# takahiroharada/OCLRadixSort

Hardware: AMD Instinct MI355X
Metric: Gkeys/s on uniform-random u32 keys; achieved % of HBM-read roofline (higher is better)
Workload: dtype u32; 1 GPU; Key-only RadixSort32, 67108864 uniform-random u32 keys (splitmix64 hi32, seed 123+step), 1xMI355X, in place; keys_per_gpu=67108864, parallelism=1 GPU, sort_algo=auto, digit_bits=8

## Files before the change

oclradixsort_amd/csrc/adlhip.hip:

```cpp
#include "../../include/adlhip.h"

#include <hip/hip_runtime.h>

#include <algorithm>
#include <cmath>
#include <cstdarg>
#include <cstdio>
#include <cstdlib>
#include <cstring>
#include <map>
#include <mutex>
#include <utility>
#include <string>
#include <vector>

#include "radix_kernels.hpp"
#include "onesweep_kernels.hpp"
#include "hybrid_kernels.hpp"
#include "persist_kernels.hpp"
#include "finish16_kernels.hpp"
#include "soa_wide_kernels.hpp"

#ifndef ADLHIP_SINGLE_TU
#define X(...) extern template __global__ __VA_ARGS__;
// ... 59 lines not shown
    uint64_t used_bytes = 0;
    int sort_algo = -1;
    int digit_bits = 8;
    int profile = 0;
    int tile_variant = -1;
    int rank_mode = 1;
    int lds_ordered = 0;
    int resident_wgs_device = 0;
    int resident_wgs = 0;
    int mid_path = 1;
    int mid_skip = 0;
    int mid2_skip = 0;
    int mid_backoff = 32, mid2_backoff = 64;
    int bin_finish = 1;
    int persist = 1;
    int msd2_path = 1;
    int net_lookback = 1;
    int partition_lookback = 1;
    int dict_path = 1;
    adlhip::DictBlock* d_dict = nullptr;
    uint32_t* d_msd2 = nullptr;
    std::vector<PendingProf> pending;
    std::vector<hipEvent_t> event_pool;
    std::map<std::string, ProfEntry> prof;
    std::vector<std::string> prof_order;
    std::vector<Staging> staging;
    std::vector<PinnedBlock> pinned_pool;
    size_t pinned_pool_bytes = 0;
    uint32_t* d_fault = nullptr;
    uint32_t* h_fault = nullptr;
// ... 524 lines not shown
    const size_t lds = std::max(own, (size_t)adlhip::TileCfg<E, 8, NT, K>::LDS_BYTES);
    if (ensure_lds(kern, lds)) return ADLHIP_FAILURE;
    const size_t per_cu = std::max<size_t>(1, std::min<size_t>((size_t)160 * 1024 / lds, (size_t)32 / (NT / 64)));
    const uint32_t grid = slab.state ? (uint32_t)num_segments
                                     : (uint32_t)std::min<size_t>(num_segments, per_cu * (size_t)d->prop.multiProcessorCount);
    return launch(d, sizeof(E) == 4 ? "segment_sort_u32" : "segment_sort_e64", [&] {
        hipLaunchKernelGGL(kern, dim3(grid), dim3(NT), lds, d->stream, in, out, seg_start, (uint32_t)num_segments, (uint32_t)low_bits,
                           dyn, d->d_fault, coop, slab);
    });
}

template <typename E, int K, typename S = E, bool SOA = false, int RANK = 1>
int launch_wave_segment_sort(adlhip_device* d, const E* in, E* out, const uint32_t* seg_start, size_t num_segments, int low_bits,
                             const uint32_t* seg_cnt = nullptr, uint32_t in_stride = 0, const uint32_t* gate = nullptr,
                             const uint32_t* dyn_low_bits = nullptr, uint32_t* out_vals = nullptr, const uint32_t* list = nullptr,
                             const uint32_t* list_cnt = nullptr, uint32_t seg_shift = 8)
{
    constexpr size_t per_wave = sizeof(E) * 64 * K + 256 * 4;
    constexpr int WAVES = per_wave <= 6144 ? 8    : per_wave <= 12288 ? 4 : per_wave <= 24576 ? 2 : 1;
    constexpr int STEP = K <= 40 ? 2 : 4;
    constexpr int RMIN = K <= 24 ? 2 : K / 2;
    const size_t lds = (size_t)WAVES * per_wave;
    if (list) {
        if constexpr (!SOA) {
            auto kern = adlhip::wave_segment_sort_kernel<E, K, WAVES, STEP, RMIN, S, SOA, true>;
            if (ensure_lds(kern, lds)) return ADLHIP_FAILURE;
            const size_t slots = std::min<size_t>(num_segments, (size_t)4 * d->prop.multiProcessorCount);
            const uint32_t grid = (uint32_t)((slots + WAVES - 1) / WAVES);
            return launch(d, sizeof(E) == 4 ? "segment_sort_listed_u32" : "segment_sort_listed_e64", [&] {
                hipLaunchKernelGGL(kern, dim3(grid), dim3(64 * WAVES), lds, d->stream, in, out, seg_start, (uint32_t)num_segments,
                                   (uint32_t)low_bits, d->d_fault, seg_cnt, in_stride, gate, dyn_low_bits, out_vals, list, list_cnt, seg_shift);
            });
        } else {
            return fail("internal: no list form for SoA");
        }
    }
    auto kern = adlhip::wave_segment_sort_kernel<E, K, WAVES, STEP, RMIN, S, SOA, false, RANK>;
    if (ensure_lds(kern, lds)) return ADLHIP_FAILURE;
    const uint32_t grid = (uint32_t)((num_segments + WAVES - 1) / WAVES);
    return launch(d, sizeof(E) == 4 ? "segment_sort_wave_u32" : "segment_sort_wave_e64", [&] {
        hipLaunchKernelGGL(kern, dim3(grid), dim3(64 * WAVES), lds, d->stream, in, out, seg_start, (uint32_t)num_segments,
                           (uint32_t)low_bits, d->d_fault, seg_cnt, in_stride, gate, dyn_low_bits, out_vals, list, list_cnt, seg_shift);
    });
}

template <typename E, typename S, int NT, int K, int BITS>
int launch_bin_segment_sort(adlhip_device* d, const S* in, E* out, const uint32_t* seg_off, const uint32_t* seg_cnt, uint32_t in_stride,
// ... 391 lines not shown
    L.off_mode = 0;
    L.off_cnt = L.off_mode + 256;
    L.off_off = L.off_cnt + 65536 * 4;
    L.off_hard = align_up(L.off_off + 65537 * 4, 256);
    L.off_coop = L.off_hard + 65536 * 4;
    L.off_slab_a = align_up(L.off_coop + kNetTableBytes, 256);
    L.off_slab_b = align_up(L.off_slab_a + (size_t)256 * L.stride_a * elem_bytes, 256);
    const size_t slab_b_bytes = (size_t)L.slots * L.stride_b * (elem_bytes == 4 && L.seg_shift == 8 ? 2 : elem_bytes);
    L.slab_b_in_tmp = elem_bytes == 4 && L.seg_shift == 8 && n >= kSlabInTmpMin && slab_b_bytes <= n * elem_bytes;
    L.total = L.off_slab_b + (L.slab_b_in_tmp ? 0 : slab_b_bytes);
    return L;
}

template <typename E, typename S, bool SOA = false>
int launch_large_finish(adlhip_device* d, const E* slab_b, E* out, uint32_t* out_vals, uint32_t* seg_off, uint32_t* seg_cnt, uint32_t stride_b,
                        uint32_t tier_b, uint32_t* mode, uint32_t* hard, int low_bits_max, bool bin, uint32_t seg_shift = 8);
bool use_bin_finish(const adlhip_device* d, size_t elem_bytes, bool key64, size_t n, bool whole_keys);

template <typename E>
int msd2_sort(adlhip_device* d, E* data, E* tmp, void* work, size_t n, int headroom_pct = kFullHeadroomPct)
{
    constexpr int K = sizeof(E) == 4 ? 32 : 16;
    constexpr int KEY_BITS = 8 * (int)sizeof(E);
    constexpr bool k32 = sizeof(E) == 4;
    uint32_t* cur_a = d->d_msd2;
    uint32_t* cur_b = d->d_msd2 + 8192;
    uint32_t* flag = d->d_msd2 + 8192 + 65536;
    uint32_t* done = flag + 1;
    uint32_t* sample = flag + 8;
    const Msd2Layout L = msd2_layout(n, sizeof(E), headroom_pct);
    char* wb = reinterpret_cast<char*>(work);
// ... 57 lines not shown
    using CC = adlhip::TileCfg<E, 8, 512, K>;
    auto ko = adlhip::msd2_offsets_kernel<E, 512, K>;
    if (ensure_lds(ko, CC::LDS_BYTES)) return ADLHIP_FAILURE;
    rc = launch(d, "msd2_offsets", [&] {
        hipLaunchKernelGGL(ko, dim3(net_wgs(d)), dim3(512), CC::LDS_BYTES, d->stream, cur_a, cur_b, flag, done, bar,
                           seg_cnt, seg_off, mode, (uint32_t)n, sample, data, tmp, ctable, d->d_fault, KEY_BITS,
                           8u - L.seg_shift, d->dict_path ? d->d_dict : nullptr, net_stats(d),
                           net_onesweep_args(d, wb + L.off_slab_a, (size_t)256 * L.stride_a * sizeof(E), n, 4, CC::TILE));
    });
    if (rc) return rc;
    using S = typename std::conditional<sizeof(E) == 4, uint16_t, E>::type;
    uint32_t* hard = reinterpret_cast<uint32_t*>(wb + L.off_hard);
    const int low_max = KEY_BITS - 8 - (int)L.seg_shift;
    const bool bin = use_bin_finish(d, sizeof(E), sizeof(E) == 8, L.seg_shift < 8 ? (size_t(24) << 20) : n, true);
    if (sizeof(E) == 4 && !slab16)
        return launch_large_finish<E, E>(d, slab_b, data, nullptr, seg_off, seg_cnt, L.stride_b, L.tier_b, mode, hard, low_max, bin, L.seg_shift);
    return launch_large_finish<E, S>(d, slab_b, data, nullptr, seg_off, seg_cnt, L.stride_b, L.tier_b, mode, hard, low_max, bin, L.seg_shift);
}

constexpr size_t kMsd2sAutoMin = size_t(1) << 20;
constexpr size_t kMsd2sMax = (size_t(1) << 28) + (size_t(1) << 22);
constexpr uint32_t msd2s_tile(size_t elem_bytes) { return elem_bytes == 8 ? 8192u : 16384u; }

struct Msd2sLayout {
    size_t off_mode, off_place, off_cnt, off_off, off_hard, off_coop, off_tickets, off_status_a, off_status_b, off_slab_a, off_slab_b, total;
    uint32_t pieces, slice, rows_a, rows_b, stride_a, stride_b, tier_b, ticket_words, seg_shift, slots;
    size_t status_bytes_a, status_bytes_b;
    bool slab_b_in_tmp;
};

Msd2sLayout msd2s_layout(size_t n, size_t elem_bytes = 8, bool slab16 = false, bool lean = false)
{
// ... 56 lines not shown
    const bool forced = d->msd2_path >= 2;
    const bool whole = sort_bits == max_bits;
    if (d->rank_mode != 1 && (keys || n > (size_t(96) << 20) || msd2_tier_b(n, 256u << msd2_seg_shift(n, false)) > 2560u)) return kLargeNone;
    if (!keys) return n > (forced ? kMsd2Min : kMsd2sAutoMin) && n <= kMsd2sMax ? kLargeStable : kLargeNone;
    if (n <= (forced || elem_bytes == 8 ? kMsd2Min : kMsd2AutoMin)) return kLargeNone;
    const size_t cursor_max = elem_bytes == 4 ? kMsd2MaxU32 : kMsd2MaxU64;
    if (!whole || d->msd2_path == 3) return n <= kMsd2sMax ? kLargeStable : kLargeNone;
    if (d->msd2_path == 4) return n <= cursor_max ? kLargeCursor : kLargeNone;
    if (d->msd2_path == 5) return n <= kMsd2sMax ? kLargeHybrid : kLargeNone;
    const size_t hybrid_min = d->persist ? (size_t(192) << 20) : (size_t(96) << 20);
    if (elem_bytes == 4 && n >= hybrid_min && n <= kMsd2sMax) return kLargeHybrid;
    if (elem_bytes == 8 && n >= (size_t(48) << 20) && n <= kMsd2sMax) return kLargeStable;
    return n <= cursor_max ? kLargeCursor : kLargeNone;
}

template <typename E, typename S, bool SOA>
int launch_large_finish(adlhip_device* d, const E* slab_b, E* out, uint32_t* out_vals, uint32_t* seg_off, uint32_t* seg_cnt, uint32_t stride_b,
                        uint32_t tier_b, uint32_t* mode, uint32_t* hard, int low_bits_max, bool bin, uint32_t seg_shift)
{
    const uint32_t* lowb = mode + adlhip::kDynLowBits;
    const size_t slots = (size_t)256 << seg_shift;
    constexpr bool wg_kind = !SOA && sizeof(E) == 4 && sizeof(S) == 2;
    if constexpr (wg_kind) {
        if (d->persist && !bin && seg_shift == 8 && tier_b <= 2560 && (stride_b & 1u) == 0u) {
            const uint16_t* sb = reinterpret_cast<const uint16_t*>(slab_b);
#define ADLHIP_F16(R2_, WAVES_)                                                                                                      \
    {                                                                                                                                \
        auto kf = adlhip::wave_finish16_kernel<R2_, WAVES_, true, true, 1>;                                                                   \
        const size_t lds = (size_t)WAVES_ * adlhip::Finish16Cfg<R2_>::PER_WAVE;                                                      \
        if (ensure_lds(kf, lds)) return ADLHIP_FAILURE;                                                                              \
        return launch(d, "segment_sort_wave_u32", [&] {                                                                              \
            hipLaunchKernelGGL(kf, dim3((uint32_t)((slots + WAVES_ - 1) / WAVES_)), dim3(64 * WAVES_), lds, d->stream, sb, out, seg_off,       \
                               seg_cnt, stride_b, mode, lowb, (uint32_t)slots, d->d_fault);                                          \
        });                                                                                                                          \
    }
            if (tier_b <= 1280) ADLHIP_F16(10, 4)
            if (tier_b <= 1536) ADLHIP_F16(12, 4)
            ADLHIP_F16(20, 4)
#undef ADLHIP_F16
        }
    }
    static const uint32_t wg_min = getenv("ADLHIP_WG_MIN_TIER") ? (uint32_t)atoi(getenv("ADLHIP_WG_MIN_TIER")) : 3072u;
    static const int wg_nt = getenv("ADLHIP_WG_NT") ? atoi(getenv("ADLHIP_WG_NT")) : 0;
    if (tier_b > 5120 || (wg_kind && tier_b >= wg_min && seg_shift == 8)) {
        if constexpr (wg_kind) {
            const S* sb = reinterpret_cast<const S*>(slab_b);
            if (seg_shift != 8) return fail("internal: the workgroup-per-segment finish takes 65536 segments");
#define ADLHIP_WG(NT_, K_) return launch_wg_segment_sort<E, S, NT_, K_>(d, sb, out, seg_off, seg_cnt, stride_b, mode, slots)
            switch (tier_b) {
            case 1280: if (wg_nt == 256) ADLHIP_WG(256, 5); ADLHIP_WG(128, 10);
            case 1536: if (wg_nt == 256) ADLHIP_WG(256, 6); ADLHIP_WG(128, 12);
            case 2560: if (wg_nt == 128) ADLHIP_WG(128, 20); ADLHIP_WG(256, 10);
            case 3072: ADLHIP_WG(256, 12);
            case 4096: ADLHIP_WG(256, 16);
// ... 139 lines not shown
        if (d->rank_mode == 0) ko = adlhip::msd2s_offsets_kernel<E, CT::TILE, 512, NK, 0, NP>;
    }
    if (ensure_lds(ko, CC::LDS_BYTES)) return ADLHIP_FAILURE;
    const adlhip::OsNet os = net_onesweep_args(d, (NP && whole && !soa_keys) ? wb + L.off_slab_a : nullptr, L.off_slab_b - L.off_slab_a, n, 4, CC::TILE);
    rc = launch(d, "msd2s_offsets", [&] {
        hipLaunchKernelGGL(ko, dim3(net_wgs(d)), dim3(512), CC::LDS_BYTES, d->stream,
                           (const uint32_t*)status_a, L.rows_a, L.slice, L.pieces, (const uint32_t*)status_b, L.rows_b, L.stride_a, flag,
                           done, bar, seg_cnt, seg_off, mode, (uint32_t)n, (const adlhip::StablePlace*)place,
                           soa_keys ? slab_a : data, soa_keys ? slab_b : tmp, ctable, d->d_fault, soa_keys, soa_vals, cur_b, 8u - L.seg_shift,
                           net_dict, net_stats(d), os);
    });
    if (rc) return rc;
    const int low_max = sort_bits - 8 - (int)L.seg_shift;
    const bool bin = use_bin_finish(d, sizeof(E), KEY64, L.seg_shift < 8 ? (size_t(24) << 20) : n, whole);
    if constexpr (k32) {
        if (slab16) return launch_large_finish<E, uint16_t>(d, slab_b, data, nullptr, seg_off, seg_cnt, L.stride_b, L.tier_b, mode, hard, low_max, bin, L.seg_shift);
        return launch_large_finish<E, E>(d, slab_b, data, nullptr, seg_off, seg_cnt, L.stride_b, L.tier_b, mode, hard, low_max, false, L.seg_shift);
    } else {
        if (soa_keys)
            return launch_large_finish<E, E, true>(d, slab_b, reinterpret_cast<E*>(soa_keys), soa_vals, seg_off, seg_cnt, L.stride_b, L.tier_b, mode,
                                                   hard, low_max, false, L.seg_shift);
        return launch_large_finish<E, E>(d, slab_b, data, nullptr, seg_off, seg_cnt, L.stride_b, L.tier_b, mode, hard, low_max, bin, L.seg_shift);
    }
}

size_t large_work_bytes(LargeForm form, size_t elem_bytes, size_t n, bool whole)
{
    if (form == kLargeCursor) return msd2_layout(n, elem_bytes).total;
    if (form == kLargeStable || form == kLargeHybrid) return msd2s_layout(n, elem_bytes, elem_bytes == 4 && whole).total;
    return 0;
}

size_t sort_work_bytes_at(const adlhip_device* d, int elem_kind, size_t n, int sort_bits, int level)
{
    const size_t a = work_bytes_three_kernel(d, n);
    if (level == 0) return a;
    size_t b;
// ... 908 lines not shown
    } else if (!strcmp(name, "sort.tile")) {
        if (value < -1 || value >= kNumVariants) return fail("sort.tile must be in [-1,%d)", kNumVariants);
        d->tile_variant = value;

    } else if (!strcmp(name, "sort.mid")) {
        if (value < 0 || value > 3) return fail("sort.mid must be 0 (off), 1 (on), 2 (keys: always the two-launch form) or 3 (always the three-launch form)");
        d->mid_path = value;
    } else if (!strcmp(name, "sort.msd2")) {
        if (value < 0 || value > 5)
            return fail("sort.msd2 must be 0 (off), 1 (on), 2 (always, from 1 Mi elements; forms by size), 3 (always the stable passes), "
                        "4 (always the cursor passes for whole keys) or 5 (always the hybrid form for whole keys)");
        d->msd2_path = value;
    } else if (!strcmp(name, "sort.persist")) {
        if (value != 0 && value != 1) return fail("sort.persist must be 0 (one tile per workgroup, round 3) or 1 (persistent prefetching passes + 16-bit finish)");
        d->persist = value;
    } else if (!strcmp(name, "sort.net_lookback")) {
        d->net_lookback = value ? 1 : 0;
    } else if (!strcmp(name, "partition.lookback")) {
        d->partition_lookback = value ? 1 : 0;
    } else if (!strcmp(name, "sort.dict")) {
        if (value != 0 && value != 1) return fail("sort.dict must be 0 (off) or 1 (counting sort for keys that take few distinct values)");
        d->dict_path = value;
    } else if (!strcmp(name, "sort.binfinish")) {
        if (value < 0 || value > 2) return fail("sort.binfinish must be 0 (LSD finish), 1 (binning finish for whole u64 keys from 24 Mi keys up) or 2 (always, u32 keys too)");
        d->bin_finish = value;
    } else if (!strcmp(name, "debug.resident_wgs")) {
        if (value < 0) return fail("debug.resident_wgs must be >= 0");
        d->resident_wgs = value ? value : d->resident_wgs_device;
    } else if (!strcmp(name, "debug.idle_poke")) {
        const int region = (int)((uint32_t)value >> 24);
// ... 16 lines not shown
    }
    return ADLHIP_SUCCESS;
}

int adlhip_get_param(adlhip_device* d, const char* name, int* value)
{
    if (!d || !name || !value) return fail("null argument");
    if (!strcmp(name, "sort.algo")) *value = d->sort_algo;
    else if (!strcmp(name, "sort.digit_bits")) *value = d->digit_bits;
    else if (!strcmp(name, "sort.tile")) *value = d->tile_variant;
    else if (!strcmp(name, "sort.rank")) *value = d->rank_mode;
    else if (!strcmp(name, "sort.mid")) *value = d->mid_path;
    else if (!strcmp(name, "sort.msd2")) *value = d->msd2_path;
    else if (!strcmp(name, "sort.binfinish")) *value = d->bin_finish;
    else if (!strcmp(name, "sort.persist")) *value = d->persist;
    else if (!strcmp(name, "sort.dict")) *value = d->dict_path;
    else if (!strcmp(name, "partition.lookback")) *value = d->partition_lookback;
    else if (!strcmp(name, "sort.net_lookback")) *value = d->net_lookback;
    else if (!strcmp(name, "debug.resident_wgs")) *value = d->resident_wgs;
    else if (!strcmp(name, "stat.net_runs") || !strcmp(name, "stat.net_counting")) {
        uint32_t v[2] = {0u, 0u};
        HIPCHK(hipMemcpyAsync(v, net_stats(d), 8, hipMemcpyDeviceToHost, d->stream));
        HIPCHK(hipStreamSynchronize(d->stream));
        *value = (int)v[name[9] == 'c' ? 1 : 0];
    }
    else if (!strcmp(name, "debug.idle_dirty") || !strcmp(name, "debug.idle_first")) {
        uint32_t dirty = 0u, first = 0u;
        if (idle_check(d, &dirty, &first)) return ADLHIP_FAILURE;
        *value = (int)(name[11] == 'd' ? dirty : first);
    }
// ... 184 lines not shown
```

oclradixsort_amd/csrc/finish16_kernels.hpp:

```cpp
#pragma once
#include <hip/hip_runtime.h>
#include <stdint.h>

#include "hybrid_kernels.hpp"

namespace adlhip {

template <int R2>
struct Finish16Cfg {
    static constexpr int CAP = 128 * R2;
    static constexpr size_t PER_WAVE = 2 * CAP + 256 * 4;
};

__device__ __forceinline__ uint32_t finish16_index(uint32_t p) { return (p & ~127u) | ((p & 63u) << 1) | ((p >> 6) & 1u); }

template <int RR, bool NTL, bool NTS, int ALG>
__device__ __forceinline__ void finish16_rows(const uint32_t* __restrict__ src32, uint32_t* __restrict__ out, uint32_t m, int lane,
                                              uint16_t* __restrict__ buf16, uint32_t* __restrict__ cnt, uint32_t low_bits, uint32_t hi)
{
    constexpr int L = RR - 1;
    const bool a_lo = 2u * (uint32_t)(64 * L + lane) < m, a_hi = 2u * (uint32_t)(64 * L + lane) + 1u < m;
    const bool b_lo = (uint32_t)(128 * L + lane) < m, b_hi = (uint32_t)(128 * L + 64 + lane) < m;
    uint32_t kp[RR];
#pragma unroll
    for (int j = 0; j < RR; ++j)
        if (j < L || a_lo) kp[j] = NTL ? __builtin_nontemporal_load(src32 + j * 64 + lane) : src32[j * 64 + lane];
    bool placed = false;
    const int npass = ((int)low_bits + 7) / 8;
    int sb = 0;
    const uint32_t* buf32 = reinterpret_cast<const uint32_t*>(buf16);
    for (int p = 0; p < npass; ++p) {
        const int nb = ((int)low_bits - sb + (npass - p - 1)) / (npass - p);
        const uint32_t mask = (1u << nb) - 1u;
        const bool v_lo = placed ? b_lo : a_lo, v_hi = placed ? b_hi : a_hi;
        auto dlo = [&](uint32_t x) -> uint32_t { return (x >> sb) & mask; };
        auto dhi = [&](uint32_t x) -> uint32_t { return (x >> (16 + sb)) & mask; };
        {
            const uint32_t d0 = (uint32_t)__builtin_amdgcn_readfirstlane((int)dlo(kp[0]));
            bool same = true;
#pragma unroll
            for (int j = 0; j < RR; ++j) {
                if (j < L || v_lo) same &= dlo(kp[j]) == d0;
                if (j < L || v_hi) same &= dhi(kp[j]) == d0;
            }
            if (__all(same)) {
                sb += nb;
                continue;
            }
        }
        const u32x4 z = {0u, 0u, 0u, 0u};
        *reinterpret_cast<u32x4*>(cnt + 4 * lane) = z;
        uint32_t rk[RR];
#pragma unroll
        for (int j = 0; j < RR; ++j) {
            if constexpr (ALG == 0) {
                if (j < L || v_lo) __hip_atomic_fetch_add(&cnt[dlo(kp[j])], 1u, __ATOMIC_RELAXED, __HIP_MEMORY_SCOPE_WAVEFRONT);
                if (j < L || v_hi) __hip_atomic_fetch_add(&cnt[dhi(kp[j])], 1u, __ATOMIC_RELAXED, __HIP_MEMORY_SCOPE_WAVEFRONT);
            } else {
                uint32_t r0 = 0u, r1 = 0u;
                if (j < L || v_lo) r0 = __hip_atomic_fetch_add(&cnt[dlo(kp[j])], 1u, __ATOMIC_RELAXED, __HIP_MEMORY_SCOPE_WAVEFRONT);
                if (j < L || v_hi) r1 = __hip_atomic_fetch_add(&cnt[dhi(kp[j])], 1u, __ATOMIC_RELAXED, __HIP_MEMORY_SCOPE_WAVEFRONT);
                rk[j] = r0 | (r1 << 16);
            }
        }
        {
            const u32x4 c = *reinterpret_cast<const u32x4*>(cnt + 4 * lane);
            const uint32_t s4 = c.x + c.y + c.z + c.w;
            const uint32_t ex = wave_incl_scan_u32(s4) - s4;
            u32x4 o;
            o.x = ex;
            o.y = ex + c.x;
            o.z = o.y + c.y;
            o.w = o.z + c.z;
            *reinterpret_cast<u32x4*>(cnt + 4 * lane) = o;
        }
        if constexpr (ALG == 0) {
#pragma unroll
            for (int j = 0; j < RR; ++j) {
                uint32_t p0 = 0u, p1 = 0u;
                if (j < L || v_lo) p0 = __hip_atomic_fetch_add(&cnt[dlo(kp[j])], 1u, __ATOMIC_RELAXED, __HIP_MEMORY_SCOPE_WAVEFRONT);
                if (j < L || v_hi) p1 = __hip_atomic_fetch_add(&cnt[dhi(kp[j])], 1u, __ATOMIC_RELAXED, __HIP_MEMORY_SCOPE_WAVEFRONT);
                if (j < L || v_lo) buf16[finish16_index(p0)] = (uint16_t)kp[j];
                if (j < L || v_hi) buf16[finish16_index(p1)] = (uint16_t)(kp[j] >> 16);
            }
        } else {
            const volatile uint32_t* start = cnt;
#pragma unroll
            for (int j = 0; j < RR; ++j) {
                uint32_t p0 = 0u, p1 = 0u;
                if (j < L || v_lo) p0 = start[dlo(kp[j])] + (rk[j] & 0xffffu);
                if (j < L || v_hi) p1 = start[dhi(kp[j])] + (rk[j] >> 16);
                if (j < L || v_lo) buf16[finish16_index(p0)] = (uint16_t)kp[j];
                if (j < L || v_hi) buf16[finish16_index(p1)] = (uint16_t)(kp[j] >> 16);
            }
        }
#pragma unroll
        for (int j = 0; j < RR; ++j)
            if (j < L || b_lo) kp[j] = buf32[j * 64 + lane];
        placed = true;
        sb += nb;
    }
    if (placed) {
#pragma unroll
        for (int j = 0; j < RR; ++j) {
            if (j < L || b_lo) {
                if constexpr (NTS) __builtin_nontemporal_store(hi | (kp[j] & 0xffffu), out + 128 * j + lane);
                else out[128 * j + lane] = hi | (kp[j] & 0xffffu);
            }
            if (j < L || b_hi) {
                if constexpr (NTS) __builtin_nontemporal_store(hi | (kp[j] >> 16), out + 128 * j + 64 + lane);
                else out[128 * j + 64 + lane] = hi | (kp[j] >> 16);
            }
        }
    } else {
#pragma unroll
        for (int j = 0; j < RR; ++j) {
            if (j < L || a_lo) out[2 * (64 * j + lane)] = hi | (kp[j] & 0xffffu);
            if (j < L || a_hi) out[2 * (64 * j + lane) + 1] = hi | (kp[j] >> 16);
        }
    }
}

template <int RR, int R2, bool NTL, bool NTS, int ALG>
__device__ __forceinline__ void finish16_dispatch(int rows2, const uint32_t* __restrict__ src32, uint32_t* __restrict__ out, uint32_t m,
                                                  int lane, uint16_t* __restrict__ buf16, uint32_t* __restrict__ cnt, uint32_t low_bits,
                                                  uint32_t hi)
{
    if constexpr (RR >= R2) {
        finish16_rows<R2, NTL, NTS, ALG>(src32, out, m, lane, buf16, cnt, low_bits, hi);
    } else {
        if (rows2 <= RR) finish16_rows<RR, NTL, NTS, ALG>(src32, out, m, lane, buf16, cnt, low_bits, hi);
        else finish16_dispatch<RR + 1, R2, NTL, NTS, ALG>(rows2, src32, out, m, lane, buf16, cnt, low_bits, hi);
    }
}

template <int R2, int WAVES, bool NTL = false, bool NTS = false, int ALG = 0>
__global__ __launch_bounds__(64 * WAVES) void wave_finish16_kernel(const uint16_t* __restrict__ slab, uint32_t* __restrict__ out,
                                                                    const uint32_t* __restrict__ seg_off,
                                                                    const uint32_t* __restrict__ seg_cnt, uint32_t stride,
                                                                    const uint32_t* __restrict__ gate, const uint32_t* __restrict__ dyn,
                                                                    uint32_t num_segments, uint32_t* fault)
{
    if (gate && *gate != 0u) return;
    using C = Finish16Cfg<R2>;
    extern __shared__ __attribute__((aligned(16))) unsigned char smem[];
    const int lane = (int)threadIdx.x & 63;
    const int w = (int)threadIdx.x >> 6;
    unsigned char* mine = smem + (size_t)w * C::PER_WAVE;
    uint16_t* __restrict__ buf16 = reinterpret_cast<uint16_t*>(mine);
    uint32_t* __restrict__ cnt = reinterpret_cast<uint32_t*>(mine + 2 * C::CAP);
    const uint32_t seg = (uint32_t)__builtin_amdgcn_readfirstlane((int)(blockIdx.x * (uint32_t)WAVES + (uint32_t)w));
    if (seg >= num_segments) return;
    const uint32_t low_bits = (uint32_t)__builtin_amdgcn_readfirstlane((int)dyn[0]);
    const uint32_t m = (uint32_t)__builtin_amdgcn_readfirstlane((int)seg_cnt[seg]);
    const uint32_t begin = (uint32_t)__builtin_amdgcn_readfirstlane((int)seg_off[seg]);
    if (m == 0u) return;
    if (m > (uint32_t)C::CAP || low_bits > 16u) {
        if (lane == 0) atomicOr(fault + 1, 0x40000u);
        return;
    }
    const uint32_t hi = ((dyn[1] << 16) | seg) << low_bits;
    const uint32_t* src32 = reinterpret_cast<const uint32_t*>(slab + (size_t)seg * stride);
    finish16_dispatch<1, R2, NTL, NTS, ALG>((int)((m + 127u) >> 7), src32, out + begin, m, lane, buf16, cnt, low_bits, hi);
}

}
```

oclradixsort_amd/csrc/finish_kernels.inc:

```
X(void adlhip::bin_segment_sort_kernel<unsigned int, unsigned int, 256, 10, 12>(unsigned int const*, unsigned int*, unsigned int const*, unsigned int const*, unsigned int, unsigned int, unsigned int const*, unsigned int*, unsigned int*, unsigned int*, unsigned int))
X(void adlhip::bin_segment_sort_kernel<unsigned int, unsigned int, 256, 6, 11>(unsigned int const*, unsigned int*, unsigned int const*, unsigned int const*, unsigned int, unsigned int, unsigned int const*, unsigned int*, unsigned int*, unsigned int*, unsigned int))
X(void adlhip::bin_segment_sort_kernel<unsigned int, unsigned int, 512, 10, 12>(unsigned int const*, unsigned int*, unsigned int const*, unsigned int const*, unsigned int, unsigned int, unsigned int const*, unsigned int*, unsigned int*, unsigned int*, unsigned int))
X(void adlhip::bin_segment_sort_kernel<unsigned int, unsigned short, 256, 10, 12>(unsigned short const*, unsigned int*, unsigned int const*, unsigned int const*, unsigned int, unsigned int, unsigned int const*, unsigned int*, unsigned int*, unsigned int*, unsigned int))
X(void adlhip::bin_segment_sort_kernel<unsigned int, unsigned short, 256, 6, 11>(unsigned short const*, unsigned int*, unsigned int const*, unsigned int const*, unsigned int, unsigned int, unsigned int const*, unsigned int*, unsigned int*, unsigned int*, unsigned int))
X(void adlhip::bin_segment_sort_kernel<unsigned int, unsigned short, 512, 10, 12>(unsigned short const*, unsigned int*, unsigned int const*, unsigned int const*, unsigned int, unsigned int, unsigned int const*, unsigned int*, unsigned int*, unsigned int*, unsigned int))
X(void adlhip::bin_segment_sort_kernel<unsigned long, unsigned long, 256, 10, 12>(unsigned long const*, unsigned long*, unsigned int const*, unsigned int const*, unsigned int, unsigned int, unsigned int const*, unsigned int*, unsigned int*, unsigned int*, unsigned int))
X(void adlhip::bin_segment_sort_kernel<unsigned long, unsigned long, 256, 6, 11>(unsigned long const*, unsigned long*, unsigned int const*, unsigned int const*, unsigned int, unsigned int, unsigned int const*, unsigned int*, unsigned int*, unsigned int*, unsigned int))
X(void adlhip::bin_segment_sort_kernel<unsigned long, unsigned long, 512, 10, 12>(unsigned long const*, unsigned long*, unsigned int const*, unsigned int const*, unsigned int, unsigned int, unsigned int const*, unsigned int*, unsigned int*, unsigned int*, unsigned int))
X(void adlhip::segment_sort_kernel<unsigned int, 256, 16, 8>(unsigned int const*, unsigned int*, unsigned int const*, unsigned int, unsigned int, unsigned int const*, unsigned int*, adlhip::MidCoop, adlhip::SegSlab))
X(void adlhip::segment_sort_kernel<unsigned int, 256, 16, 9>(unsigned int const*, unsigned int*, unsigned int const*, unsigned int, unsigned int, unsigned int const*, unsigned int*, adlhip::MidCoop, adlhip::SegSlab))
X(void adlhip::segment_sort_kernel<unsigned int, 512, 16, 8>(unsigned int const*, unsigned int*, unsigned int const*, unsigned int, unsigned int, unsigned int const*, unsigned int*, adlhip::MidCoop, adlhip::SegSlab))
X(void adlhip::segment_sort_kernel<unsigned int, 512, 16, 9>(unsigned int const*, unsigned int*, unsigned int const*, unsigned int, unsigned int, unsigned int const*, unsigned int*, adlhip::MidCoop, adlhip::SegSlab))
X(void adlhip::segment_sort_kernel<unsigned int, 512, 32, 8>(unsigned int const*, unsigned int*, unsigned int const*, unsigned int, unsigned int, unsigned int const*, unsigned int*, adlhip::MidCoop, adlhip::SegSlab))
X(void adlhip::segment_sort_kernel<unsigned long, 256, 16, 8>(unsigned long const*, unsigned long*, unsigned int const*, unsigned int, unsigned int, unsigned int const*, unsigned int*, adlhip::MidCoop, adlhip::SegSlab))
X(void adlhip::segment_sort_kernel<unsigned long, 256, 16, 9>(unsigned long const*, unsigned long*, unsigned int const*, unsigned int, unsigned int, unsigned int const*, unsigned int*, adlhip::MidCoop, adlhip::SegSlab))
X(void adlhip::segment_sort_kernel<unsigned long, 512, 16, 8>(unsigned long const*, unsigned long*, unsigned int const*, unsigned int, unsigned int, unsigned int const*, unsigned int*, adlhip::MidCoop, adlhip::SegSlab))
X(void adlhip::wave_finish16_kernel<10, 4, true, true, 1>(unsigned short const*, unsigned int*, unsigned int const*, unsigned int const*, unsigned int, unsigned int const*, unsigned int const*, unsigned int, unsigned int*))
X(void adlhip::wave_finish16_kernel<12, 4, true, true, 1>(unsigned short const*, unsigned int*, unsigned int const*, unsigned int const*, unsigned int, unsigned int const*, unsigned int const*, unsigned int, unsigned int*))
X(void adlhip::wave_finish16_kernel<20, 4, true, true, 1>(unsigned short const*, unsigned int*, unsigned int const*, unsigned int const*, unsigned int, unsigned int const*, unsigned int const*, unsigned int, unsigned int*))
X(void adlhip::wg_segment_sort_kernel<unsigned int, unsigned short, 128, 10>(unsigned short const*, unsigned int*, unsigned int const*, unsigned int const*, unsigned int, unsigned int const*, unsigned int const*, unsigned int*))
X(void adlhip::wg_segment_sort_kernel<unsigned int, unsigned short, 128, 12>(unsigned short const*, unsigned int*, unsigned int const*, unsigned int const*, unsigned int, unsigned int const*, unsigned int const*, unsigned int*))
X(void adlhip::wg_segment_sort_kernel<unsigned int, unsigned short, 128, 20>(unsigned short const*, unsigned int*, unsigned int const*, unsigned int const*, unsigned int, unsigned int const*, unsigned int const*, unsigned int*))
X(void adlhip::wg_segment_sort_kernel<unsigned int, unsigned short, 256, 10>(unsigned short const*, unsigned int*, unsigned int const*, unsigned int const*, unsigned int, unsigned int const*, unsigned int const*, unsigned int*))
X(void adlhip::wg_segment_sort_kernel<unsigned int, unsigned short, 256, 12>(unsigned short const*, unsigned int*, unsigned int const*, unsigned int const*, unsigned int, unsigned int const*, unsigned int const*, unsigned int*))
X(void adlhip::wg_segment_sort_kernel<unsigned int, unsigned short, 256, 16>(unsigned short const*, unsigned int*, unsigned int const*, unsigned int const*, unsigned int, unsigned int const*, unsigned int const*, unsigned int*))
X(void adlhip::wg_segment_sort_kernel<unsigned int, unsigned short, 256, 20>(unsigned short const*, unsigned int*, unsigned int const*, unsigned int const*, unsigned int, unsigned int const*, unsigned int const*, unsigned int*))
X(void adlhip::wg_segment_sort_kernel<unsigned int, unsigned short, 256, 32>(unsigned short const*, unsigned int*, unsigned int const*, unsigned int const*, unsigned int, unsigned int const*, unsigned int const*, unsigned int*))
X(void adlhip::wg_segment_sort_kernel<unsigned int, unsigned short, 256, 48>(unsigned short const*, unsigned int*, unsigned int const*, unsigned int const*, unsigned int, unsigned int const*, unsigned int const*, unsigned int*))
X(void adlhip::wg_segment_sort_kernel<unsigned int, unsigned short, 256, 5>(unsigned short const*, unsigned int*, unsigned int const*, unsigned int const*, unsigned int, unsigned int const*, unsigned int const*, unsigned int*))
X(void adlhip::wg_segment_sort_kernel<unsigned int, unsigned short, 256, 6>(unsigned short const*, unsigned int*, unsigned int const*, unsigned int const*, unsigned int, unsigned int const*, unsigned int const*, unsigned int*))
X(void adlhip::wg_segment_sort_kernel<unsigned int, unsigned short, 512, 10>(unsigned short const*, unsigned int*, unsigned int const*, unsigned int const*, unsigned int, unsigned int const*, unsigned int const*, unsigned int*))
X(void adlhip::wg_segment_sort_kernel<unsigned int, unsigned short, 512, 16>(unsigned short const*, unsigned int*, unsigned int const*, unsigned int const*, unsigned int, unsigned int const*, unsigned int const*, unsigned int*))
X(void adlhip::wg_segment_sort_kernel<unsigned int, unsigned short, 512, 24>(unsigned short const*, unsigned int*, unsigned int const*, unsigned int const*, unsigned int, unsigned int const*, unsigned int const*, unsigned int*))
X(void adlhip::wg_segment_sort_kernel<unsigned int, unsigned short, 512, 32>(unsigned short const*, unsigned int*, unsigned int const*, unsigned int const*, unsigned int, unsigned int const*, unsigned int const*, unsigned int*))
// ... 2 lines not shown
```

Baseline: 208.1 Gkeys/s.

## Size 16-bit finish kernel rows from n and spill oversized segments to listed sort

The 16-bit wave finish now picks its row-pair capacity from the expected segment size (mean plus three standard deviations) instead of the slab tier, so the main kernel uses less LDS and fewer registers for typical segments. Segments that exceed this smaller capacity are appended to a hard list and sorted by a second listed wave-segment-sort launch queued back to back. The row dispatch also starts near the expected size and skips bounds checks on non-final rows. Wavefront fences replace a volatile read in the rank path. The cost is an extra launch and a risk that tail segments go through the slower fallback.

Result: slower. 204.7 Gkeys/s (-1.6%).

```diff
diff --git a/oclradixsort_amd/csrc/adlhip.hip b/oclradixsort_amd/csrc/adlhip.hip
--- a/oclradixsort_amd/csrc/adlhip.hip
+++ b/oclradixsort_amd/csrc/adlhip.hip
@@ -97,6 +97,7 @@
     int mid_backoff = 32, mid2_backoff = 64;
     int bin_finish = 1;
     int persist = 1;
+    int finish_rows = 0;
     int msd2_path = 1;
     int net_lookback = 1;
     int partition_lookback = 1;
@@ -651,7 +652,7 @@
 int launch_wave_segment_sort(adlhip_device* d, const E* in, E* out, const uint32_t* seg_start, size_t num_segments, int low_bits,
                              const uint32_t* seg_cnt = nullptr, uint32_t in_stride = 0, const uint32_t* gate = nullptr,
                              const uint32_t* dyn_low_bits = nullptr, uint32_t* out_vals = nullptr, const uint32_t* list = nullptr,
-                             const uint32_t* list_cnt = nullptr, uint32_t seg_shift = 8)
+                             const uint32_t* list_cnt = nullptr, uint32_t seg_shift = 8, bool inside_launch = false)
 {
     constexpr size_t per_wave = sizeof(E) * 64 * K + 256 * 4;
     constexpr int WAVES = per_wave <= 6144 ? 8    : per_wave <= 12288 ? 4 : per_wave <= 24576 ? 2 : 1;
@@ -664,10 +665,15 @@
             if (ensure_lds(kern, lds)) return ADLHIP_FAILURE;
             const size_t slots = std::min<size_t>(num_segments, (size_t)4 * d->prop.multiProcessorCount);
             const uint32_t grid = (uint32_t)((slots + WAVES - 1) / WAVES);
-            return launch(d, sizeof(E) == 4 ? "segment_sort_listed_u32" : "segment_sort_listed_e64", [&] {
+            auto enqueue = [&] {
                 hipLaunchKernelGGL(kern, dim3(grid), dim3(64 * WAVES), lds, d->stream, in, out, seg_start, (uint32_t)num_segments,
                                    (uint32_t)low_bits, d->d_fault, seg_cnt, in_stride, gate, dyn_low_bits, out_vals, list, list_cnt, seg_shift);
-            });
+            };
+            if (inside_launch) {
+                enqueue();
+                return ADLHIP_SUCCESS;
+            }
+            return launch(d, sizeof(E) == 4 ? "segment_sort_listed_u32" : "segment_sort_listed_e64", enqueue);
         } else {
             return fail("internal: no list form for SoA");
         }
@@ -1089,7 +1095,7 @@
 
 template <typename E, typename S, bool SOA = false>
 int launch_large_finish(adlhip_device* d, const E* slab_b, E* out, uint32_t* out_vals, uint32_t* seg_off, uint32_t* seg_cnt, uint32_t stride_b,
-                        uint32_t tier_b, uint32_t* mode, uint32_t* hard, int low_bits_max, bool bin, uint32_t seg_shift = 8);
+                        uint32_t tier_b, uint32_t* mode, uint32_t* hard, int low_bits_max, bool bin, uint32_t seg_shift, size_t n);
 bool use_bin_finish(const adlhip_device* d, size_t elem_bytes, bool key64, size_t n, bool whole_keys);
 
 template <typename E>
@@ -1177,8 +1183,8 @@
     const int low_max = KEY_BITS - 8 - (int)L.seg_shift;
     const bool bin = use_bin_finish(d, sizeof(E), sizeof(E) == 8, L.seg_shift < 8 ? (size_t(24) << 20) : n, true);
     if (sizeof(E) == 4 && !slab16)
-        return launch_large_finish<E, E>(d, slab_b, data, nullptr, seg_off, seg_cnt, L.stride_b, L.tier_b, mode, hard, low_max, bin, L.seg_shift);
-    return launch_large_finish<E, S>(d, slab_b, data, nullptr, seg_off, seg_cnt, L.stride_b, L.tier_b, mode, hard, low_max, bin, L.seg_shift);
+        return launch_large_finish<E, E>(d, slab_b, data, nullptr, seg_off, seg_cnt, L.stride_b, L.tier_b, mode, hard, low_max, bin, L.seg_shift, n);
+    return launch_large_finish<E, S>(d, slab_b, data, nullptr, seg_off, seg_cnt, L.stride_b, L.tier_b, mode, hard, low_max, bin, L.seg_shift, n);
 }
 
 constexpr size_t kMsd2sAutoMin = size_t(1) << 20;
@@ -1265,9 +1271,22 @@
     return n <= cursor_max ? kLargeCursor : kLargeNone;
 }
 
+int finish16_main_rows(const adlhip_device* d, size_t n, int tier_r2)
+{
+    size_t r = (size_t)d->finish_rows;
+    if (d->finish_rows <= 0) {
+        const size_t mean = (n + 65535) / 65536;
+        size_t sd = 1;
+        while (sd * sd < mean) ++sd;
+        r = (mean + 3 * sd + 127) / 128;
+    }
+    r = r <= 6 ? 6 : r <= 12 ? r : (r + 1) / 2 * 2;
+    return (int)std::min<size_t>(r, (size_t)tier_r2);
+}
+
 template <typename E, typename S, bool SOA>
 int launch_large_finish(adlhip_device* d, const E* slab_b, E* out, uint32_t* out_vals, uint32_t* seg_off, uint32_t* seg_cnt, uint32_t stride_b,
-                        uint32_t tier_b, uint32_t* mode, uint32_t* hard, int low_bits_max, bool bin, uint32_t seg_shift)
+                        uint32_t tier_b, uint32_t* mode, uint32_t* hard, int low_bits_max, bool bin, uint32_t seg_shift, size_t n)
 {
     const uint32_t* lowb = mode + adlhip::kDynLowBits;
     const size_t slots = (size_t)256 << seg_shift;
@@ -1275,20 +1294,36 @@
     if constexpr (wg_kind) {
         if (d->persist && !bin && seg_shift == 8 && tier_b <= 2560 && (stride_b & 1u) == 0u) {
             const uint16_t* sb = reinterpret_cast<const uint16_t*>(slab_b);
-#define ADLHIP_F16(R2_, WAVES_)                                                                                                      \
-    {                                                                                                                                \
-        auto kf = adlhip::wave_finish16_kernel<R2_, WAVES_, true, true, 1>;                                                                   \
-        const size_t lds = (size_t)WAVES_ * adlhip::Finish16Cfg<R2_>::PER_WAVE;                                                      \
-        if (ensure_lds(kf, lds)) return ADLHIP_FAILURE;                                                                              \
-        return launch(d, "segment_sort_wave_u32", [&] {                                                                              \
-            hipLaunchKernelGGL(kf, dim3((uint32_t)((slots + WAVES_ - 1) / WAVES_)), dim3(64 * WAVES_), lds, d->stream, sb, out, seg_off,       \
-                               seg_cnt, stride_b, mode, lowb, (uint32_t)slots, d->d_fault);                                          \
-        });                                                                                                                          \
-    }
-            if (tier_b <= 1280) ADLHIP_F16(10, 4)
-            if (tier_b <= 1536) ADLHIP_F16(12, 4)
-            ADLHIP_F16(20, 4)
+            const int tier_r2 = (int)(tier_b <= 1280 ? 10 : tier_b <= 1536 ? 12 : 20);
+            const int r_main = finish16_main_rows(d, n, tier_r2);
+            void (*kf)(const uint16_t*, uint32_t*, const uint32_t*, const uint32_t*, uint32_t, const uint32_t*, const uint32_t*, uint32_t,
+                       uint32_t*, uint32_t, uint32_t*, uint32_t*) = nullptr;
+            size_t lds = 0;
+            switch (r_main) {
+#define ADLHIP_F16(R2_)                                                      \
+    case R2_:                                                                \
+        kf = adlhip::wave_finish16_kernel<R2_, 4, true, true, 1>;           \
+        lds = (size_t)4 * adlhip::Finish16Cfg<R2_>::PER_WAVE;               \
+        break;
+                ADLHIP_F16(6) ADLHIP_F16(7) ADLHIP_F16(8) ADLHIP_F16(9) ADLHIP_F16(10) ADLHIP_F16(11) ADLHIP_F16(12)
+                ADLHIP_F16(14) ADLHIP_F16(16) ADLHIP_F16(18) ADLHIP_F16(20)
 #undef ADLHIP_F16
+            default: return fail("internal: no 16-bit finish of %d row pairs", r_main);
+            }
+            if (ensure_lds(kf, lds)) return ADLHIP_FAILURE;
+            uint32_t* hc = mode + adlhip::kDynHardCnt;
+            int rc_list = ADLHIP_SUCCESS;
+            const int rc = launch(d, "segment_sort_wave_u32", [&] {
+                hipLaunchKernelGGL(kf, dim3((uint32_t)((slots + 3) / 4)), dim3(256), lds, d->stream, sb, out, seg_off, seg_cnt, stride_b, mode,
+                                   lowb, (uint32_t)slots, d->d_fault, tier_b, hc, hard);
+                if (tier_b <= kMsd2Stride0)
+                    rc_list = launch_wave_segment_sort<E, kMsd2Stride0 / 64, S>(d, slab_b, out, seg_off, slots, low_bits_max, seg_cnt, stride_b, mode,
+                                                                               lowb, nullptr, hard, hc, seg_shift, true);
+                else
+                    rc_list = launch_wave_segment_sort<E, 40, S>(d, slab_b, out, seg_off, slots, low_bits_max, seg_cnt, stride_b, mode, lowb,
+                                                                 nullptr, hard, hc, seg_shift, true);
+            });
+            return rc ? rc : rc_list;
         }
     }
     static const uint32_t wg_min = getenv("ADLHIP_WG_MIN_TIER") ? (uint32_t)atoi(getenv("ADLHIP_WG_MIN_TIER")) : 3072u;
@@ -1458,13 +1493,13 @@
     const int low_max = sort_bits - 8 - (int)L.seg_shift;
     const bool bin = use_bin_finish(d, sizeof(E), KEY64, L.seg_shift < 8 ? (size_t(24) << 20) : n, whole);
     if constexpr (k32) {
-        if (slab16) return launch_large_finish<E, uint16_t>(d, slab_b, data, nullptr, seg_off, seg_cnt, L.stride_b, L.tier_b, mode, hard, low_max, bin, L.seg_shift);
-        return launch_large_finish<E, E>(d, slab_b, data, nullptr, seg_off, seg_cnt, L.stride_b, L.tier_b, mode, hard, low_max, false, L.seg_shift);
+        if (slab16) return launch_large_finish<E, uint16_t>(d, slab_b, data, nullptr, seg_off, seg_cnt, L.stride_b, L.tier_b, mode, hard, low_max, bin, L.seg_shift, n);
+        return launch_large_finish<E, E>(d, slab_b, data, nullptr, seg_off, seg_cnt, L.stride_b, L.tier_b, mode, hard, low_max, false, L.seg_shift, n);
     } else {
         if (soa_keys)
             return launch_large_finish<E, E, true>(d, slab_b, reinterpret_cast<E*>(soa_keys), soa_vals, seg_off, seg_cnt, L.stride_b, L.tier_b, mode,
-                                                   hard, low_max, false, L.seg_shift);
-        return launch_large_finish<E, E>(d, slab_b, data, nullptr, seg_off, seg_cnt, L.stride_b, L.tier_b, mode, hard, low_max, bin, L.seg_shift);
+                                                   hard, low_max, false, L.seg_shift, n);
+        return launch_large_finish<E, E>(d, slab_b, data, nullptr, seg_off, seg_cnt, L.stride_b, L.tier_b, mode, hard, low_max, bin, L.seg_shift, n);
     }
 }
 
@@ -2403,6 +2438,11 @@
     } else if (!strcmp(name, "sort.persist")) {
         if (value != 0 && value != 1) return fail("sort.persist must be 0 (one tile per workgroup, round 3) or 1 (persistent prefetching passes + 16-bit finish)");
         d->persist = value;
+    } else if (!strcmp(name, "sort.finish_rows")) {
+        if (value < 0 || value > 20)
+            return fail("sort.finish_rows must be 0 (from n) or 1 ... 20 (row pairs of 128 keys the 16-bit finish's main launch holds; "
+                        "from the slab tier's own count up: one tier)");
+        d->finish_rows = value;
     } else if (!strcmp(name, "sort.net_lookback")) {
         d->net_lookback = value ? 1 : 0;
     } else if (!strcmp(name, "partition.lookback")) {
@@ -2449,6 +2489,7 @@
     else if (!strcmp(name, "sort.msd2")) *value = d->msd2_path;
     else if (!strcmp(name, "sort.binfinish")) *value = d->bin_finish;
     else if (!strcmp(name, "sort.persist")) *value = d->persist;
+    else if (!strcmp(name, "sort.finish_rows")) *value = d->finish_rows;
     else if (!strcmp(name, "sort.dict")) *value = d->dict_path;
     else if (!strcmp(name, "partition.lookback")) *value = d->partition_lookback;
     else if (!strcmp(name, "sort.net_lookback")) *value = d->net_lookback;
diff --git a/oclradixsort_amd/csrc/finish16_kernels.hpp b/oclradixsort_amd/csrc/finish16_kernels.hpp
--- a/oclradixsort_amd/csrc/finish16_kernels.hpp
+++ b/oclradixsort_amd/csrc/finish16_kernels.hpp
@@ -14,17 +14,21 @@
 
 __device__ __forceinline__ uint32_t finish16_index(uint32_t p) { return (p & ~127u) | ((p & 63u) << 1) | ((p >> 6) & 1u); }
 
-template <int RR, bool NTL, bool NTS, int ALG>
+__device__ __forceinline__ void finish16_fence() { __builtin_amdgcn_fence(__ATOMIC_ACQ_REL, "wavefront"); }
+
+template <int RR, bool ALL, bool NTL, bool NTS, int ALG>
 __device__ __forceinline__ void finish16_rows(const uint32_t* __restrict__ src32, uint32_t* __restrict__ out, uint32_t m, int lane,
                                               uint16_t* __restrict__ buf16, uint32_t* __restrict__ cnt, uint32_t low_bits, uint32_t hi)
 {
     constexpr int L = RR - 1;
-    const bool a_lo = 2u * (uint32_t)(64 * L + lane) < m, a_hi = 2u * (uint32_t)(64 * L + lane) + 1u < m;
-    const bool b_lo = (uint32_t)(128 * L + lane) < m, b_hi = (uint32_t)(128 * L + 64 + lane) < m;
+    auto a_lo = [&](int j) -> bool { return (!ALL && j < L) || (uint32_t)(128 * j + 2 * lane) < m; };
+    auto a_hi = [&](int j) -> bool { return (!ALL && j < L) || (uint32_t)(128 * j + 2 * lane) + 1u < m; };
+    auto b_lo = [&](int j) -> bool { return (!ALL && j < L) || (uint32_t)(128 * j + lane) < m; };
+    auto b_hi = [&](int j) -> bool { return (!ALL && j < L) || (uint32_t)(128 * j + 64 + lane) < m; };
     uint32_t kp[RR];
 #pragma unroll
     for (int j = 0; j < RR; ++j)
-        if (j < L || a_lo) kp[j] = NTL ? __builtin_nontemporal_load(src32 + j * 64 + lane) : src32[j * 64 + lane];
+        if (a_lo(j)) kp[j] = NTL ? __builtin_nontemporal_load(src32 + j * 64 + lane) : src32[j * 64 + lane];
     bool placed = false;
     const int npass = ((int)low_bits + 7) / 8;
     int sb = 0;
@@ -32,7 +36,8 @@
     for (int p = 0; p < npass; ++p) {
         const int nb = ((int)low_bits - sb + (npass - p - 1)) / (npass - p);
         const uint32_t mask = (1u << nb) - 1u;
-        const bool v_lo = placed ? b_lo : a_lo, v_hi = placed ? b_hi : a_hi;
+        auto v_lo = [&](int j) -> bool { return placed ? b_lo(j) : a_lo(j); };
+        auto v_hi = [&](int j) -> bool { return placed ? b_hi(j) : a_hi(j); };
         auto dlo = [&](uint32_t x) -> uint32_t { return (x >> sb) & mask; };
         auto dhi = [&](uint32_t x) -> uint32_t { return (x >> (16 + sb)) & mask; };
         {
@@ -40,8 +45,8 @@
             bool same = true;
 #pragma unroll
             for (int j = 0; j < RR; ++j) {
-                if (j < L || v_lo) same &= dlo(kp[j]) == d0;
-                if (j < L || v_hi) same &= dhi(kp[j]) == d0;
+                if (v_lo(j)) same &= dlo(kp[j]) == d0;
+                if (v_hi(j)) same &= dhi(kp[j]) == d0;
             }
             if (__all(same)) {
                 sb += nb;
@@ -50,19 +55,21 @@
         }
         const u32x4 z = {0u, 0u, 0u, 0u};
         *reinterpret_cast<u32x4*>(cnt + 4 * lane) = z;
+        finish16_fence();
         uint32_t rk[RR];
 #pragma unroll
         for (int j = 0; j < RR; ++j) {
             if constexpr (ALG == 0) {
-                if (j < L || v_lo) __hip_atomic_fetch_add(&cnt[dlo(kp[j])], 1u, __ATOMIC_RELAXED, __HIP_MEMORY_SCOPE_WAVEFRONT);
-                if (j < L || v_hi) __hip_atomic_fetch_add(&cnt[dhi(kp[j])], 1u, __ATOMIC_RELAXED, __HIP_MEMORY_SCOPE_WAVEFRONT);
+                if (v_lo(j)) __hip_atomic_fetch_add(&cnt[dlo(kp[j])], 1u, __ATOMIC_RELAXED, __HIP_MEMORY_SCOPE_WAVEFRONT);
+                if (v_hi(j)) __hip_atomic_fetch_add(&cnt[dhi(kp[j])], 1u, __ATOMIC_RELAXED, __HIP_MEMORY_SCOPE_WAVEFRONT);
             } else {
                 uint32_t r0 = 0u, r1 = 0u;
-                if (j < L || v_lo) r0 = __hip_atomic_fetch_add(&cnt[dlo(kp[j])], 1u, __ATOMIC_RELAXED, __HIP_MEMORY_SCOPE_WAVEFRONT);
-                if (j < L || v_hi) r1 = __hip_atomic_fetch_add(&cnt[dhi(kp[j])], 1u, __ATOMIC_RELAXED, __HIP_MEMORY_SCOPE_WAVEFRONT);
+                if (v_lo(j)) r0 = __hip_atomic_fetch_add(&cnt[dlo(kp[j])], 1u, __ATOMIC_RELAXED, __HIP_MEMORY_SCOPE_WAVEFRONT);
+                if (v_hi(j)) r1 = __hip_atomic_fetch_add(&cnt[dhi(kp[j])], 1u, __ATOMIC_RELAXED, __HIP_MEMORY_SCOPE_WAVEFRONT);
                 rk[j] = r0 | (r1 << 16);
             }
         }
+        finish16_fence();
         {
             const u32x4 c = *reinterpret_cast<const u32x4*>(cnt + 4 * lane);
             const uint32_t s4 = c.x + c.y + c.z + c.w;
@@ -74,40 +81,42 @@
             o.w = o.z + c.z;
             *reinterpret_cast<u32x4*>(cnt + 4 * lane) = o;
         }
+        finish16_fence();
         if constexpr (ALG == 0) {
 #pragma unroll
             for (int j = 0; j < RR; ++j) {
                 uint32_t p0 = 0u, p1 = 0u;
-                if (j < L || v_lo) p0 = __hip_atomic_fetch_add(&cnt[dlo(kp[j])], 1u, __ATOMIC_RELAXED, __HIP_MEMORY_SCOPE_WAVEFRONT);
-                if (j < L || v_hi) p1 = __hip_atomic_fetch_add(&cnt[dhi(kp[j])], 1u, __ATOMIC_RELAXED, __HIP_MEMORY_SCOPE_WAVEFRONT);
-                if (j < L || v_lo) buf16[finish16_index(p0)] = (uint16_t)kp[j];
-                if (j < L || v_hi) buf16[finish16_index(p1)] = (uint16_t)(kp[j] >> 16);
+                if (v_lo(j)) p0 = __hip_atomic_fetch_add(&cnt[dlo(kp[j])], 1u, __ATOMIC_RELAXED, __HIP_MEMORY_SCOPE_WAVEFRONT);
+                if (v_hi(j)) p1 = __hip_atomic_fetch_add(&cnt[dhi(kp[j])], 1u, __ATOMIC_RELAXED, __HIP_MEMORY_SCOPE_WAVEFRONT);
+                if (v_lo(j)) buf16[finish16_index(p0)] = (uint16_t)kp[j];
+                if (v_hi(j)) buf16[finish16_index(p1)] = (uint16_t)(kp[j] >> 16);
             }
         } else {
-            const volatile uint32_t* start = cnt;
+            const uint32_t* start = cnt;
 #pragma unroll
             for (int j = 0; j < RR; ++j) {
                 uint32_t p0 = 0u, p1 = 0u;
-                if (j < L || v_lo) p0 = start[dlo(kp[j])] + (rk[j] & 0xffffu);
-                if (j < L || v_hi) p1 = start[dhi(kp[j])] + (rk[j] >> 16);
-                if (j < L || v_lo) buf16[finish16_index(p0)] = (uint16_t)kp[j];
-                if (j < L || v_hi) buf16[finish16_index(p1)] = (uint16_t)(kp[j] >> 16);
+                if (v_lo(j)) p0 = start[dlo(kp[j])] + (rk[j] & 0xffffu);
+                if (v_hi(j)) p1 = start[dhi(kp[j])] + (rk[j] >> 16);
+                if (v_lo(j)) buf16[finish16_index(p0)] = (uint16_t)kp[j];
+                if (v_hi(j)) buf16[finish16_index(p1)] = (uint16_t)(kp[j] >> 16);
             }
         }
+        finish16_fence();
 #pragma unroll
         for (int j = 0; j < RR; ++j)
-            if (j < L || b_lo) kp[j] = buf32[j * 64 + lane];
+            if (b_lo(j)) kp[j] = buf32[j * 64 + lane];
         placed = true;
         sb += nb;
     }
     if (placed) {
 #pragma unroll
         for (int j = 0; j < RR; ++j) {
-            if (j < L || b_lo) {
+            if (b_lo(j)) {
                 if constexpr (NTS) __builtin_nontemporal_store(hi | (kp[j] & 0xffffu), out + 128 * j + lane);
                 else out[128 * j + lane] = hi | (kp[j] & 0xffffu);
             }
-            if (j < L || b_hi) {
+            if (b_hi(j)) {
                 if constexpr (NTS) __builtin_nontemporal_store(hi | (kp[j] >> 16), out + 128 * j + 64 + lane);
                 else out[128 * j + 64 + lane] = hi | (kp[j] >> 16);
             }
@@ -115,22 +124,23 @@
     } else {
 #pragma unroll
         for (int j = 0; j < RR; ++j) {
-            if (j < L || a_lo) out[2 * (64 * j + lane)] = hi | (kp[j] & 0xffffu);
-            if (j < L || a_hi) out[2 * (64 * j + lane) + 1] = hi | (kp[j] >> 16);
+            if (a_lo(j)) out[2 * (64 * j + lane)] = hi | (kp[j] & 0xffffu);
+            if (a_hi(j)) out[2 * (64 * j + lane) + 1] = hi | (kp[j] >> 16);
         }
     }
 }
 
-template <int RR, int R2, bool NTL, bool NTS, int ALG>
+template <int RR, int R2, bool FIRST, bool NTL, bool NTS, int ALG>
 __device__ __forceinline__ void finish16_dispatch(int rows2, const uint32_t* __restrict__ src32, uint32_t* __restrict__ out, uint32_t m,
                                                   int lane, uint16_t* __restrict__ buf16, uint32_t* __restrict__ cnt, uint32_t low_bits,
                                                   uint32_t hi)
 {
+    constexpr bool ALL = FIRST && RR > 1;
     if constexpr (RR >= R2) {
-        finish16_rows<R2, NTL, NTS, ALG>(src32, out, m, lane, buf16, cnt, low_bits, hi);
+        finish16_rows<R2, ALL, NTL, NTS, ALG>(src32, out, m, lane, buf16, cnt, low_bits, hi);
     } else {
-        if (rows2 <= RR) finish16_rows<RR, NTL, NTS, ALG>(src32, out, m, lane, buf16, cnt, low_bits, hi);
-        else finish16_dispatch<RR + 1, R2, NTL, NTS, ALG>(rows2, src32, out, m, lane, buf16, cnt, low_bits, hi);
+        if (rows2 <= RR) finish16_rows<RR, ALL, NTL, NTS, ALG>(src32, out, m, lane, buf16, cnt, low_bits, hi);
+        else finish16_dispatch<RR + 1, R2, false, NTL, NTS, ALG>(rows2, src32, out, m, lane, buf16, cnt, low_bits, hi);
     }
 }
 
@@ -139,10 +149,12 @@
                                                                     const uint32_t* __restrict__ seg_off,
                                                                     const uint32_t* __restrict__ seg_cnt, uint32_t stride,
                                                                     const uint32_t* __restrict__ gate, const uint32_t* __restrict__ dyn,
-                                                                    uint32_t num_segments, uint32_t* fault)
+                                                                    uint32_t num_segments, uint32_t* fault, uint32_t cap,
+                                                                    uint32_t* hard_cnt, uint32_t* hard_list)
 {
     if (gate && *gate != 0u) return;
     using C = Finish16Cfg<R2>;
+    constexpr int RLO = R2 <= 6 ? 1 : R2 <= 12 ? R2 - 3 : R2 - 5;
     extern __shared__ __attribute__((aligned(16))) unsigned char smem[];
     const int lane = (int)threadIdx.x & 63;
     const int w = (int)threadIdx.x >> 6;
@@ -155,13 +167,17 @@
     const uint32_t m = (uint32_t)__builtin_amdgcn_readfirstlane((int)seg_cnt[seg]);
     const uint32_t begin = (uint32_t)__builtin_amdgcn_readfirstlane((int)seg_off[seg]);
     if (m == 0u) return;
-    if (m > (uint32_t)C::CAP || low_bits > 16u) {
+    if (m > cap || low_bits > 16u) {
         if (lane == 0) atomicOr(fault + 1, 0x40000u);
+        return;
+    }
+    if (m > (uint32_t)C::CAP) {
+        if (lane == 0) hard_list[__hip_atomic_fetch_add(hard_cnt, 1u, __ATOMIC_RELAXED, __HIP_MEMORY_SCOPE_AGENT)] = seg;
         return;
     }
     const uint32_t hi = ((dyn[1] << 16) | seg) << low_bits;
     const uint32_t* src32 = reinterpret_cast<const uint32_t*>(slab + (size_t)seg * stride);
-    finish16_dispatch<1, R2, NTL, NTS, ALG>((int)((m + 127u) >> 7), src32, out + begin, m, lane, buf16, cnt, low_bits, hi);
+    finish16_dispatch<RLO, R2, true, NTL, NTS, ALG>((int)((m + 127u) >> 7), src32, out + begin, m, lane, buf16, cnt, low_bits, hi);
 }
 
 }
diff --git a/oclradixsort_amd/csrc/finish_kernels.inc b/oclradixsort_amd/csrc/finish_kernels.inc
--- a/oclradixsort_amd/csrc/finish_kernels.inc
+++ b/oclradixsort_amd/csrc/finish_kernels.inc
@@ -15,9 +15,17 @@
 X(void adlhip::segment_sort_kernel<unsigned long, 256, 16, 8>(unsigned long const*, unsigned long*, unsigned int const*, unsigned int, unsigned int, unsigned int const*, unsigned int*, adlhip::MidCoop, adlhip::SegSlab))
 X(void adlhip::segment_sort_kernel<unsigned long, 256, 16, 9>(unsigned long const*, unsigned long*, unsigned int const*, unsigned int, unsigned int, unsigned int const*, unsigned int*, adlhip::MidCoop, adlhip::SegSlab))
 X(void adlhip::segment_sort_kernel<unsigned long, 512, 16, 8>(unsigned long const*, unsigned long*, unsigned int const*, unsigned int, unsigned int, unsigned int const*, unsigned int*, adlhip::MidCoop, adlhip::SegSlab))
-X(void adlhip::wave_finish16_kernel<10, 4, true, true, 1>(unsigned short const*, unsigned int*, unsigned int const*, unsigned int const*, unsigned int, unsigned int const*, unsigned int const*, unsigned int, unsigned int*))
-X(void adlhip::wave_finish16_kernel<12, 4, true, true, 1>(unsigned short const*, unsigned int*, unsigned int const*, unsigned int const*, unsigned int, unsigned int const*, unsigned int const*, unsigned int, unsigned int*))
-X(void adlhip::wave_finish16_kernel<20, 4, true, true, 1>(unsigned short const*, unsigned int*, unsigned int const*, unsigned int const*, unsigned int, unsigned int const*, unsigned int const*, unsigned int, unsigned int*))
+X(void adlhip::wave_finish16_kernel<10, 4, true, true, 1>(unsigned short const*, unsigned int*, unsigned int const*, unsigned int const*, unsigned int, unsigned int const*, unsigned int const*, unsigned int, unsigned int*, unsigned int, unsigned int*, unsigned int*))
+X(void adlhip::wave_finish16_kernel<11, 4, true, true, 1>(unsigned short const*, unsigned int*, unsigned int const*, unsigned int const*, unsigned int, unsigned int const*, unsigned int const*, unsigned int, unsigned int*, unsigned int, unsigned int*, unsigned int*))
+X(void adlhip::wave_finish16_kernel<12, 4, true, true, 1>(unsigned short const*, unsigned int*, unsigned int const*, unsigned int const*, unsigned int, unsigned int const*, unsigned int const*, unsigned int, unsigned int*, unsigned int, unsigned int*, unsigned int*))
+X(void adlhip::wave_finish16_kernel<14, 4, true, true, 1>(unsigned short const*, unsigned int*, unsigned int const*, unsigned int const*, unsigned int, unsigned int const*, unsigned int const*, unsigned int, unsigned int*, unsigned int, unsigned int*, unsigned int*))
+X(void adlhip::wave_finish16_kernel<16, 4, true, true, 1>(unsigned short const*, unsigned int*, unsigned int const*, unsigned int const*, unsigned int, unsigned int const*, unsigned int const*, unsigned int, unsigned int*, unsigned int, unsigned int*, unsigned int*))
+X(void adlhip::wave_finish16_kernel<18, 4, true, true, 1>(unsigned short const*, unsigned int*, unsigned int const*, unsigned int const*, unsigned int, unsigned int const*, unsigned int const*, unsigned int, unsigned int*, unsigned int, unsigned int*, unsigned int*))
+X(void adlhip::wave_finish16_kernel<20, 4, true, true, 1>(unsigned short const*, unsigned int*, unsigned int const*, unsigned int const*, unsigned int, unsigned int const*, unsigned int const*, unsigned int, unsigned int*, unsigned int, unsigned int*, unsigned int*))
+X(void adlhip::wave_finish16_kernel<6, 4, true, true, 1>(unsigned short const*, unsigned int*, unsigned int const*, unsigned int const*, unsigned int, unsigned int const*, unsigned int const*, unsigned int, unsigned int*, unsigned int, unsigned int*, unsigned int*))
+X(void adlhip::wave_finish16_kernel<7, 4, true, true, 1>(unsigned short const*, unsigned int*, unsigned int const*, unsigned int const*, unsigned int, unsigned int const*, unsigned int const*, unsigned int, unsigned int*, unsigned int, unsigned int*, unsigned int*))
+X(void adlhip::wave_finish16_kernel<8, 4, true, true, 1>(unsigned short const*, unsigned int*, unsigned int const*, unsigned int const*, unsigned int, unsigned int const*, unsigned int const*, unsigned int, unsigned int*, unsigned int, unsigned int*, unsigned int*))
+X(void adlhip::wave_finish16_kernel<9, 4, true, true, 1>(unsigned short const*, unsigned int*, unsigned int const*, unsigned int const*, unsigned int, unsigned int const*, unsigned int const*, unsigned int, unsigned int*, unsigned int, unsigned int*, unsigned int*))
 X(void adlhip::wg_segment_sort_kernel<unsigned int, unsigned short, 128, 10>(unsigned short const*, unsigned int*, unsigned int const*, unsigned int const*, unsigned int, unsigned int const*, unsigned int const*, unsigned int*))
 X(void adlhip::wg_segment_sort_kernel<unsigned int, unsigned short, 128, 12>(unsigned short const*, unsigned int*, unsigned int const*, unsigned int const*, unsigned int, unsigned int const*, unsigned int const*, unsigned int*))
 X(void adlhip::wg_segment_sort_kernel<unsigned int, unsigned short, 128, 20>(unsigned short const*, unsigned int*, unsigned int const*, unsigned int const*, unsigned int, unsigned int const*, unsigned int const*, unsigned int*))
```
